# genomematt/xenomapper

Hardware: AMD Instinct MI355X
Metric: read-pairs/sec classified (higher is better)
Workload: dtype int32; 1 GPU; configs[1]: 50000000 PE 2x150 pairs/GPU, AS/XS, liberal, HBM-resident; pairs_per_gpu=50000000, step=xm_classify_compact_dev: classify+count, scan, scatter (3 launches)

## Files before the change

### xenomapper_amd/csrc/xm_kernels.hip

```cpp
#include <hip/hip_runtime.h>
#include <stdint.h>
#include <stdlib.h>

#include "xm_kernels.h"

namespace xm {

template <typename T>
__device__ __forceinline__ uint32_t mapping_state(T a1, T x1, T a2, T x2, T m)
{
    const bool low1 = a1 <= m;
    const bool low2 = a2 <= m;
    const bool prim = (a1 > m) && (low2 || a1 > a2);
    const bool sec  = (a2 > m) && (low1 || a2 > a1);
    const bool spec1 = (x1 == T(0)) || (a1 > x1);
    const bool spec2 = (x2 == T(0)) || (a2 > x2);
    uint32_t s = 6u;
    s = sec ? (spec2 ? 1u : 3u) : s;
    s = (a1 == a2) ? 4u : s;
    s = prim ? (spec1 ? 0u : 2u) : s;
    s = (low1 && low2) ? 5u : s;
    return s;
}

template <>
__device__ __forceinline__ uint32_t mapping_state<int32_t>(int32_t a1, int32_t x1, int32_t a2, int32_t x2, int32_t m)
{
    const bool low1 = a1 <= m, low2 = a2 <= m;
    const bool gt = a1 > a2, lt = a2 > a1;
    const bool spec1 = (x1 == 0) || (a1 > x1);
    const bool spec2 = (x2 == 0) || (a2 > x2);
    uint32_t s = spec2 ? 1u : 3u;
    s = (gt || lt) ? s : 4u;
    s = (!low1 && (low2 || gt)) ? (spec1 ? 0u : 2u) : s;
    s = (low1 && low2) ? 5u : s;
    return s;
}

__device__ __forceinline__ uint32_t bin_of_code(int mode, uint32_t c)
{
    const uint32_t f = (c >> 3) & 7u, r = c & 7u;
    const uint32_t lo = f < r ? f : r;
    const uint32_t hi = f < r ? r : f;
    uint32_t b;
    if (mode == XM_MODE_SE) {
        b = r > 6u ? 6u : r;
    } else if (mode == XM_MODE_PE_LIBERAL) {
        b = lo;
    } else {
        b = (hi == 5u) ? 5u
          : ((hi == 4u) || (((f ^ r) & 1u) != 0u)) ? 4u
          : lo;
    }
    if (mode != XM_MODE_SE) b = (hi > 5u) ? 6u : b;
    return (c == XM_NO_UNIT) ? 7u : b;
}

template <typename T> struct Vec4;
typedef int32_t v4i32 __attribute__((ext_vector_type(4)));
typedef int32_t v4i32_a4 __attribute__((ext_vector_type(4), aligned(4)));
typedef double  v4f64 __attribute__((ext_vector_type(4)));
template <> struct Vec4<int32_t> { typedef v4i32 type; };
template <> struct Vec4<double>  { typedef v4f64 type; };

template <typename T> __device__ __forceinline__ T absent_value();
template <> __device__ __forceinline__ int32_t absent_value<int32_t>() { return INT32_MIN; }
template <> __device__ __forceinline__ double  absent_value<double>()  { return -__builtin_huge_val(); }

template <typename T, bool NT, bool FULL = false>
__device__ __forceinline__ void load4(const T *__restrict__ col, uint64_t r0, uint64_t n, T out[4])
{
    typedef typename Vec4<T>::type V;
    if (FULL || r0 + 4 <= n) {
        const V *p = reinterpret_cast<const V *>(col + r0);
        const V v = NT ? __builtin_nontemporal_load(p) : *p;
        out[0] = v.x; out[1] = v.y; out[2] = v.z; out[3] = v.w;
    } else {
#pragma unroll
        for (int j = 0; j < 4; ++j) out[j] = (r0 + j < n) ? col[r0 + j] : absent_value<T>();
    }
}

template <typename T, bool NT>
__device__ __forceinline__ void load4_wg(const T *__restrict__ wg, uint32_t byte_off, T out[4])
{
    typedef typename Vec4<T>::type V;
    const V *p = reinterpret_cast<const V *>(reinterpret_cast<const char *>(wg) + byte_off);
    const V v = NT ? __builtin_nontemporal_load(p) : *p;
    out[0] = v.x; out[1] = v.y; out[2] = v.z; out[3] = v.w;
}

__device__ __forceinline__ uint32_t wave_scan_incl(uint32_t v)
{
    v += (uint32_t)__builtin_amdgcn_update_dpp(0, (int)v, 0x111, 0xf, 0xf, false);
    v += (uint32_t)__builtin_amdgcn_update_dpp(0, (int)v, 0x112, 0xf, 0xf, false);
    v += (uint32_t)__builtin_amdgcn_update_dpp(0, (int)v, 0x114, 0xf, 0xf, false);
    v += (uint32_t)__builtin_amdgcn_update_dpp(0, (int)v, 0x118, 0xf, 0xf, false);
    v += (uint32_t)__builtin_amdgcn_update_dpp(0, (int)v, 0x142, 0xa, 0xf, false);
    v += (uint32_t)__builtin_amdgcn_update_dpp(0, (int)v, 0x143, 0xc, 0xf, false);
    return v;
}

__device__ __forceinline__ uint32_t lane_value(uint32_t v, int lane)
{
    return (uint32_t)__builtin_amdgcn_readlane((int)v, lane);
}

__device__ __forceinline__ void lds_settle()
{
    asm volatile("s_waitcnt lgkmcnt(0)" ::: "memory");
}

#define XM_HREP 8
#define XM_COUNT_LDS_WORDS (64 * XM_HREP + 16)

struct CountSink {
    uint32_t *gran_counts;
    uint32_t *part_tot;
    unsigned long long *counts_rep;
    uint8_t *bins4;
    uint32_t gran_stride;
    int mode;
    uint32_t blk0;
};

__device__ __forceinline__ void count_flush(uint32_t *lds, uint32_t granule, const CountSink &sink)
{
    const uint32_t lane = threadIdx.x & 63u;
    uint32_t *misc = lds + 64 * XM_HREP;
    const uint4 h0 = *reinterpret_cast<const uint4 *>(lds + lane * XM_HREP);
    const uint4 h1 = *reinterpret_cast<const uint4 *>(lds + lane * XM_HREP + 4);
    const uint32_t s = h0.x + h0.y + h0.z + h0.w + h1.x + h1.y + h1.z + h1.w;
    if (s != 0u) {
        atomicAdd(&sink.counts_rep[(granule % XM_COUNT_REPLICAS) * 64u + lane], (unsigned long long)s);
        atomicAdd(&misc[8u + bin_of_code(sink.mode, lane)], s);
    }
    lds_settle();
    if (lane < 8u) {
        const uint32_t v = misc[8u + lane];
        sink.gran_counts[(uint64_t)lane * sink.gran_stride + granule] = v;
        if (v != 0u) atomicAdd(&sink.part_tot[((granule & (XM_PART_REPLICAS - 1u)) * 8u + lane) * XM_PART_STRIDE + granule / XM_PART_GRAN], v);
    }
}

template <int BLOCK>
__device__ __forceinline__ void count_units(const uint32_t c[4], uint32_t *lds, const CountSink &sink)
{
    const uint32_t lane = threadIdx.x & 63u;
    const uint32_t rep = lane & (XM_HREP - 1u);
#pragma unroll
    for (int j = 0; j < 4; ++j) {
        const bool unit = c[j] != XM_NO_UNIT;
        if (__ballot(unit) == 0ull) continue;
        if (unit) atomicAdd(&lds[(c[j] & 63u) * XM_HREP + rep], 1u);
    }
    lds_settle();
    uint32_t arrived = 0;
    if (lane == 0u) arrived = atomicAdd(&lds[64 * XM_HREP], 1u);
    arrived = (uint32_t)__builtin_amdgcn_readfirstlane((int)arrived);
    if (arrived != (uint32_t)(BLOCK / 64 - 1)) return;
    lds_settle();
    count_flush(lds, blockIdx.x + sink.blk0, sink);
}

template <int MODE, bool HAS6>
__device__ __forceinline__ uint32_t unit_bin(uint32_t c)
{
    if (MODE == XM_MODE_SE) return c == XM_NO_UNIT ? 7u : (c & 7u);
    const uint32_t f = (c >> 3) & 7u, r = c & 7u;
    const uint32_t lo = f < r ? f : r, hi = f < r ? r : f;
    uint32_t b = lo;
    if (MODE == XM_MODE_PE_CONSERVATIVE) {
        b = (((f ^ r) & 1u) != 0u || hi == 4u) ? 4u : b;
        b = (hi == 5u) ? 5u : b;
    }
    if (HAS6) b = (hi > 5u) ? 6u : b;
    return c == XM_NO_UNIT ? 7u : b;
}

template <int MODE, bool HAS6>
__device__ __forceinline__ uint32_t unit_bin_of(uint32_t f, uint32_t r, bool unit)
{
    uint32_t b;
    if (MODE == XM_MODE_SE) {
        b = r;
    } else {
        const uint32_t lo = f < r ? f : r, hi = f < r ? r : f;
        b = lo;
        if (MODE == XM_MODE_PE_CONSERVATIVE) {
            b = (((f ^ r) & 1u) != 0u || hi == 4u) ? 4u : b;
            b = (hi == 5u) ? 5u : b;
        }
        if (HAS6) b = (hi > 5u) ? 6u : b;
    }
    return unit ? b : 7u;
}

template <typename T, bool PAIRED, int BLOCK, bool FULL, bool COUNTS, int BINMODE>
__device__ __forceinline__ void classify_finish(const T a1[4], const T x1[4], const T a2[4], const T x2[4], T m,
                                                uint32_t mb, uint32_t halo, uint32_t *last_state,
                                                uint8_t *__restrict__ code, uint64_t r0, uint64_t n,
                                                uint32_t *count_lds, const CountSink &sink)
{
    const uint32_t lane = threadIdx.x & 63u;
    const uint32_t wave = threadIdx.x >> 6;
    uint32_t s[4];
#pragma unroll
    for (int j = 0; j < 4; ++j) s[j] = mapping_state<T>(a1[j], x1[j], a2[j], x2[j], m);

    uint32_t c[4], fwd[4] = {0, 0, 0, 0};
    if (PAIRED) {
        uint32_t prev = (uint32_t)__builtin_amdgcn_update_dpp(0, (int)s[3], 0x138, 0xf, 0xf, false);
        if (lane == 63) last_state[wave] = s[3];
        __syncthreads();
        if (lane == 0) prev = (wave == 0) ? halo : last_state[wave - 1];
        c[0] = (mb & 1u) ? ((prev << 3) | s[0]) : XM_NO_UNIT;
        c[1] = (mb & 2u) ? ((s[0] << 3) | s[1]) : XM_NO_UNIT;
        c[2] = (mb & 4u) ? ((s[1] << 3) | s[2]) : XM_NO_UNIT;
        c[3] = (mb & 8u) ? ((s[2] << 3) | s[3]) : XM_NO_UNIT;
        fwd[0] = prev; fwd[1] = s[0]; fwd[2] = s[1]; fwd[3] = s[2];
    } else {
        if (COUNTS) __syncthreads();
#pragma unroll
        for (int j = 0; j < 4; ++j) c[j] = ((mb >> j) & 1u) ? s[j] : XM_NO_UNIT;
    }

    if (FULL || r0 + 4 <= n) {
        if (code != nullptr) *reinterpret_cast<uint32_t *>(code + r0) = c[0] | (c[1] << 8) | (c[2] << 16) | (c[3] << 24);
    } else {
#pragma unroll
        for (int j = 0; j < 4; ++j)
            if (code != nullptr && r0 + j < n) code[r0 + j] = (uint8_t)c[j];
    }
    if (BINMODE >= 0) {
        uint32_t nib = 0;
#pragma unroll
        for (int j = 0; j < 4; ++j) nib |= unit_bin_of<BINMODE, sizeof(T) == 8>(fwd[j], s[j], ((mb >> j) & 1u) != 0u) << (4 * j);
        reinterpret_cast<uint16_t *>(sink.bins4)[r0 >> 2] = (uint16_t)nib;
    }
    if (COUNTS) count_units<BLOCK>(c, count_lds, sink);
}

template <typename T, bool PAIRED, bool NT, int BLOCK, bool FULL, bool COUNTS, int BINMODE>
__device__ __forceinline__ void classify_body(const T *__restrict__ as1, const T *__restrict__ xs1,
                                              const T *__restrict__ as2, const T *__restrict__ xs2,
                                              const uint8_t *__restrict__ unit_bits8, T m,
                                              uint8_t *__restrict__ code, uint64_t n, uint32_t *last_state,
                                              uint32_t *count_lds, const CountSink &sink)
{
    const uint64_t g = (uint64_t)(blockIdx.x + sink.blk0) * BLOCK + threadIdx.x;
    const uint64_t r0 = g * 4;

    T a1[4], x1[4], a2[4], x2[4];
    load4<T, NT, FULL>(as1, r0, n, a1);
    load4<T, NT, FULL>(xs1, r0, n, x1);
    load4<T, NT, FULL>(as2, r0, n, a2);
    load4<T, NT, FULL>(xs2, r0, n, x2);
    uint32_t mb = 0;
    if (FULL || r0 < n) mb = (uint32_t)(unit_bits8[g >> 1] >> ((g & 1u) * 4u)) & 0xFu;
    if (!FULL && r0 + 4 > n) mb &= (r0 < n) ? ((1u << (uint32_t)(n - r0)) - 1u) : 0u;

    uint32_t halo = 0;
    if (PAIRED && threadIdx.x == 0) {
        if (r0 > 0) {
            const uint64_t h = r0 - 1;
            halo = mapping_state<T>(as1[h], xs1[h], as2[h], xs2[h], m);
        } else {
            mb &= ~1u;
        }
    }
    classify_finish<T, PAIRED, BLOCK, FULL, COUNTS, BINMODE>(a1, x1, a2, x2, m, mb, halo, last_state, code, r0, n, count_lds, sink);
}

template <int BLOCK>
__device__ __forceinline__ void count_lds_clear(uint32_t *count_lds)
{
    for (uint32_t k = threadIdx.x; k < (uint32_t)XM_COUNT_LDS_WORDS; k += BLOCK) count_lds[k] = 0;
}

template <typename T, bool PAIRED, bool NT, int BLOCK, bool COUNTS, int BINMODE>
__global__ void __launch_bounds__(BLOCK)
classify_kernel(const T *__restrict__ as1, const T *__restrict__ xs1,
                const T *__restrict__ as2, const T *__restrict__ xs2,
                const uint8_t *__restrict__ unit_bits8, T m,
                uint8_t *__restrict__ code, uint64_t n, CountSink sink)
{
    __shared__ uint32_t last_state[BLOCK / 64];
    __shared__ __attribute__((aligned(16))) uint32_t count_lds[COUNTS ? XM_COUNT_LDS_WORDS : 4];
    if (COUNTS) count_lds_clear<BLOCK>(count_lds);
    if (((uint64_t)blockIdx.x + sink.blk0 + 1) * (BLOCK * 4) <= n)
        classify_body<T, PAIRED, NT, BLOCK, true, COUNTS, BINMODE>(as1, xs1, as2, xs2, unit_bits8, m, code, n, last_state, count_lds, sink);
    else
        classify_body<T, PAIRED, NT, BLOCK, false, COUNTS, BINMODE>(as1, xs1, as2, xs2, unit_bits8, m, code, n, last_state, count_lds, sink);
}


__device__ __attribute__((noinline)) uint4 load_codes16_tail(const uint8_t *__restrict__ code, uint64_t base, uint64_t n)
{
    uint32_t w[4];
    for (int k = 0; k < 4; ++k) {
        uint32_t acc = 0;
        for (int j = 0; j < 4; ++j) {
            const uint64_t i = base + 4 * k + j;
            const uint32_t c = (i < n) ? (uint32_t)code[i] : XM_NO_UNIT;
            acc |= c << (8 * j);
        }
        w[k] = acc;
    }
    return make_uint4(w[0], w[1], w[2], w[3]);
}

__device__ __forceinline__ void load_codes16(const uint8_t *__restrict__ code, uint64_t base, uint64_t n,
                                             uint32_t w[4])
{
    uint4 v;
    if (base + 16 <= n) v = *reinterpret_cast<const uint4 *>(code + base);
    else v = load_codes16_tail(code, base, n);
    w[0] = v.x; w[1] = v.y; w[2] = v.z; w[3] = v.w;
}

__device__ __attribute__((noinline)) uint32_t load_codes4_tail(const uint8_t *__restrict__ code, uint64_t base, uint64_t n)
{
    uint32_t acc = 0;
    for (int j = 0; j < 4; ++j) {
        const uint64_t i = base + j;
        const uint32_t c = (i < n) ? (uint32_t)code[i] : XM_NO_UNIT;
        acc |= c << (8 * j);
    }
    return acc;
}

__global__ void __launch_bounds__(XM_BLOCK)
hist_kernel(const uint8_t *__restrict__ code, uint64_t n, uint32_t n_gran, CountSink sink)
{
    __shared__ __attribute__((aligned(16))) uint32_t lds_all[XM_BLOCK / 64][XM_COUNT_LDS_WORDS];
    const uint32_t lane = threadIdx.x & 63u, wave = threadIdx.x >> 6;
    uint32_t *lds = lds_all[wave];
    const uint32_t g = blockIdx.x * (XM_BLOCK / 64) + wave;
    if (g >= n_gran) return;
    for (uint32_t k = lane; k < (uint32_t)XM_COUNT_LDS_WORDS; k += 64u) lds[k] = 0;

    constexpr int TILES = XM_GRAN / 1024;
    const uint64_t rec0 = (uint64_t)g * XM_GRAN;
    uint32_t w[TILES][4];
#pragma unroll
    for (int k = 0; k < TILES; ++k) load_codes16(code, rec0 + (uint64_t)k * 1024u + lane * 16u, n, w[k]);
    lds_settle();

    const uint32_t rep = lane & (XM_HREP - 1u);
    uint32_t common = w[0][0] & 0xFFu;
    if (common == XM_NO_UNIT) common = (w[0][0] >> 8) & 0xFFu;
    common = (uint32_t)__builtin_amdgcn_readfirstlane((int)common);
    uint32_t n_common = 0;
#pragma unroll
    for (int k = 0; k < TILES; ++k) {
#pragma unroll
        for (int j = 0; j < 16; ++j) {
            const uint32_t c = (w[k][j >> 2] >> (8 * (j & 3))) & 0xFFu;
            const bool unit = c != XM_NO_UNIT;
            if (__ballot(unit) == 0ull) continue;
            const bool same = unit && c == common;
            n_common += same ? 1u : 0u;
            if (unit && !same) atomicAdd(&lds[(c & 63u) * XM_HREP + rep], 1u);
        }
    }
    if (n_common) atomicAdd(&lds[(common & 63u) * XM_HREP + rep], n_common);
    lds_settle();
    count_flush(lds, g, sink);
}

#define XM_SCAN_THREADS 1024
__device__ __forceinline__ unsigned long long block_sum_1024(unsigned long long v, unsigned long long *wsum)
{
    v += __shfl_xor(v, 1, 64);  v += __shfl_xor(v, 2, 64);  v += __shfl_xor(v, 4, 64);
    v += __shfl_xor(v, 8, 64);  v += __shfl_xor(v, 16, 64); v += __shfl_xor(v, 32, 64);
    if ((threadIdx.x & 63u) == 0u) wsum[threadIdx.x >> 6] = v;
    __syncthreads();
    unsigned long long total = 0;
#pragma unroll
    for (int w = 0; w < XM_SCAN_THREADS / 64; ++w) total += wsum[w];
    return total;
}

__global__ void __launch_bounds__(XM_SCAN_THREADS)
scan_kernel(const uint32_t *__restrict__ gran_counts, uint32_t n_gran, uint32_t gran_stride,
            const uint32_t *__restrict__ part_tot, uint32_t *__restrict__ gran_off,
            unsigned long long *__restrict__ bin_totals,
            unsigned long long *__restrict__ counts_rep, unsigned long long *__restrict__ counts, uint32_t part0, uint32_t n_parts)
{
    __shared__ unsigned long long wsum[XM_SCAN_THREADS / 64];
    __shared__ uint32_t wtot[XM_SCAN_THREADS / 64];
    const uint32_t p = blockIdx.x + part0, b = blockIdx.y;
    const uint32_t t = threadIdx.x, lane = t & 63u, wave = t >> 6;
    if (p + 1u == n_parts && t < 64u) {
        const uint32_t slot = b * 8u + (t >> 3), part = t & 7u;
        unsigned long long acc = 0;
        for (uint32_t r = part; r < XM_COUNT_REPLICAS; r += 8u) {
            acc += counts_rep[r * 64u + slot];
            counts_rep[r * 64u + slot] = 0;
        }
        acc += __shfl_xor(acc, 1, 64);
        acc += __shfl_xor(acc, 2, 64);
        acc += __shfl_xor(acc, 4, 64);
        if (part == 0) counts[slot] = acc;
    }
    const uint32_t g = p * XM_PART_GRAN + t;
    const uint32_t x = (g < n_gran) ? gran_counts[(uint64_t)b * gran_stride + g] : 0u;
    unsigned long long part_sum = 0;
    for (uint32_t e = t; e < p * XM_PART_REPLICAS; e += XM_SCAN_THREADS) {
        const uint32_t r = e / p, q = e - r * p;
        part_sum += part_tot[(r * 8u + b) * XM_PART_STRIDE + q];
    }
    const unsigned long long carry = block_sum_1024(part_sum, wsum);

    const uint32_t incl = wave_scan_incl(x);
    if (lane == 63u) wtot[wave] = incl;
    __syncthreads();
    uint32_t before_wave = 0, part_total = 0;
    for (uint32_t w = 0; w < XM_SCAN_THREADS / 64; ++w) {
        const uint32_t v = wtot[w];
        before_wave += (w < wave) ? v : 0u;
        part_total += v;
    }
    if (g < n_gran) gran_off[(uint64_t)b * gran_stride + g] = (uint32_t)carry + before_wave + incl - x;
    if (p + 1u == n_parts && t == 0u) bin_totals[b] = carry + part_total;
}

#ifndef XM_SCATTER_GUARD
#define XM_SCATTER_GUARD 1
#endif
__device__ __forceinline__ uint32_t mbcnt64(uint64_t mask, uint32_t add)
{
    return __builtin_amdgcn_mbcnt_hi((uint32_t)(mask >> 32), __builtin_amdgcn_mbcnt_lo((uint32_t)mask, add));
}

template <bool WIDE>
__device__ __forceinline__ void store_index(uint32_t *__restrict__ idx_out, uint32_t pos, uint32_t rec)
{
    if (WIDE) idx_out[pos] = rec;
    else *reinterpret_cast<uint32_t *>(reinterpret_cast<char *>(idx_out) + (pos << 2)) = rec;
}

template <int SLOTS, bool WIDE, bool STAGED, bool LISTS = false>
__device__ __forceinline__ void scatter_256(const uint32_t bin[4], const uint32_t rec[4], uint32_t base[7],
                                            uint32_t *__restrict__ idx_out, uint32_t n_units, uint16_t *slab,
                                            const uint64_t *lptr = nullptr)
{
    uint32_t pos[4] = {0, 0, 0, 0};
#pragma unroll
    for (int b = 0; b < 7; ++b) {
        uint64_t m[4], any = 0;
#pragma unroll
        for (int j = 0; j < 4; ++j) {
            m[j] = ((SLOTS >> j) & 1) ? __ballot(bin[j] == (uint32_t)b) : 0ull;
            any |= m[j];
        }
        if (any == 0ull) continue;
        uint32_t t = base[b];
#pragma unroll
        for (int j = 0; j < 4; ++j)
            if ((SLOTS >> j) & 1) t = mbcnt64(m[j], t);
#pragma unroll
        for (int j = 0; j < 4; ++j)
            if ((SLOTS >> j) & 1) pos[j] = (bin[j] == (uint32_t)b) ? t : pos[j];
        uint32_t total = 0;
#pragma unroll
        for (int j = 0; j < 4; ++j)
            if ((SLOTS >> j) & 1) total += (uint32_t)__builtin_popcountll(m[j]);
        base[b] += total;
    }
#pragma unroll
    for (int j = 1; j < 4; ++j)
#pragma unroll
        for (int i = 0; i < j; ++i)
            if (((SLOTS >> j) & 1) && ((SLOTS >> i) & 1)) pos[j] += (bin[i] == bin[j]) ? 1u : 0u;
#pragma unroll
    for (int j = 0; j < 4; ++j)
        if (((SLOTS >> j) & 1) && bin[j] < 7u && (!XM_SCATTER_GUARD || pos[j] < n_units)) {
            if (STAGED) slab[pos[j]] = (uint16_t)rec[j];
            else if (LISTS) {
                uint32_t *list = reinterpret_cast<uint32_t *>(lptr[bin[j]]);
                if (list != nullptr) list[pos[j]] = rec[j];
            }
            else store_index<WIDE>(idx_out, pos[j], rec[j]);
        }
}

#ifndef XM_SCATTER_STAGED
#define XM_SCATTER_STAGED 1
#endif
#define XM_SLAB_U16 (XM_GRAN + 64)
#ifndef XM_STAGE_MIN_UNITS
#define XM_STAGE_MIN_UNITS 1536
#endif

template <bool WIDE>
__device__ __forceinline__ void store_index4(uint32_t *__restrict__ idx_out, uint32_t pos, uint32_t r0, uint32_t r1, uint32_t r2, uint32_t r3)
{
    typedef uint32_t v4u32_a4 __attribute__((ext_vector_type(4), aligned(4)));
    v4u32_a4 v; v.x = r0; v.y = r1; v.z = r2; v.w = r3;
    if (WIDE) *reinterpret_cast<v4u32_a4 *>(idx_out + pos) = v;
    else *reinterpret_cast<v4u32_a4 *>(reinterpret_cast<char *>(idx_out) + (pos << 2)) = v;
}

template <bool WIDE>
__device__ __forceinline__ void scatter_copy_out(const uint16_t *slab, uint32_t L, uint32_t G, uint32_t N, uint32_t rec_g,
                                                 uint32_t *__restrict__ idx_out)
{
    const uint32_t lane = threadIdx.x & 63u;
    if (N < 64u) {
        if (lane < N) store_index<WIDE>(idx_out, G + lane, rec_g + slab[L + lane]);
        return;
    }
    const uint32_t h = (0u - G) & 3u;
    const uint32_t body = (N - h) >> 2;
    const uint32_t t = (N - h) & 3u;
    {
        const bool head = lane < h, tail = lane >= 4u && lane - 4u < t;
        const uint32_t e = head ? lane : h + 4u * body + (lane - 4u);
        if (head || tail) store_index<WIDE>(idx_out, G + e, rec_g + slab[L + e]);
    }
    for (uint32_t c = lane; c < body; c += 64u) {
        const uint32_t e = h + 4u * c;
        const uint2 w = *reinterpret_cast<const uint2 *>(slab + L + e);
        store_index4<WIDE>(idx_out, G + e, rec_g + (w.x & 0xFFFFu), rec_g + (w.x >> 16), rec_g + (w.y & 0xFFFFu), rec_g + (w.y >> 16));
    }
}

template <int NSUB, bool WIDE, bool NIB, bool STAGED, bool LISTS>
__device__ __forceinline__ void scatter_granule(const uint32_t w[NSUB], const uint8_t *lut, uint32_t rec_g, uint32_t base[7],
                                                uint32_t *__restrict__ idx_out, uint32_t n_units, uint16_t *slab, const uint64_t *lptr)
{
    const uint32_t lane = threadIdx.x & 63u;
#pragma unroll
    for (int s = 0; s < NSUB; ++s) {
        const uint32_t rec0 = (STAGED ? 0u : rec_g) + (uint32_t)s * 256u + lane * 4u;
        const uint32_t limit = STAGED ? (uint32_t)XM_SLAB_U16 : n_units;
        uint32_t bin[4];
        bool even_free;
        if (NIB) {
#pragma unroll
            for (int j = 0; j < 4; ++j) bin[j] = (w[s] >> (4 * j)) & 7u;
            even_free = (w[s] & 0x0707u) == 0x0707u;
        } else {
            even_free = (w[s] & 0x00FF00FFu) == 0x00FF00FFu;
        }
        const uint32_t rec[4] = {rec0, rec0 + 1u, rec0 + 2u, rec0 + 3u};
        if (__ballot(!even_free) == 0ull) {
            if (!NIB) { bin[0] = bin[2] = 7u; bin[1] = lut[(w[s] >> 8) & 63u]; bin[3] = lut[(w[s] >> 24) & 63u]; }
            scatter_256<0xA, WIDE, STAGED, LISTS && !STAGED>(bin, rec, base, idx_out, limit, slab, lptr);
            continue;
        }
        if (!NIB) {
#pragma unroll
            for (int j = 0; j < 4; ++j) bin[j] = lut[(w[s] >> (8 * j)) & 63u];
        }
        uint32_t y;
        if (NIB) {
            const uint32_t x = w[s] ^ 0x7777u;
            y = (x | (x >> 1) | (x >> 2)) & 0x1111u;
        } else {
            y = (bin[0] < 7u ? 1u : 0u) | (bin[1] < 7u ? 0x10u : 0u) | (bin[2] < 7u ? 0x100u : 0u) | (bin[3] < 7u ? 0x1000u : 0u);
        }
        if (!STAGED && __ballot(__builtin_popcount(y) > 2) == 0ull) {
            const uint32_t rest = y & (y - 1u);
            const uint32_t c0 = y ? (uint32_t)__builtin_ctz(y) : 0u, c1 = rest ? (uint32_t)__builtin_ctz(rest) : 0u;
            const uint32_t j0 = c0 >> 2, j1 = c1 >> 2;
            uint32_t vb[4] = {7u, 7u, 7u, 7u};
            if (NIB) {
                vb[0] = y ? (w[s] >> c0) & 7u : 7u;
                vb[1] = rest ? (w[s] >> c1) & 7u : 7u;
            } else {
#pragma unroll
                for (int j = 0; j < 4; ++j) {
                    vb[0] = (y && j0 == (uint32_t)j) ? bin[j] : vb[0];
                    vb[1] = (rest && j1 == (uint32_t)j) ? bin[j] : vb[1];
                }
            }
            const uint32_t vrec[4] = {rec0 + j0, rec0 + j1, 0u, 0u};
            scatter_256<0x3, WIDE, STAGED, LISTS>(vb, vrec, base, idx_out, limit, slab, lptr);
        } else {
            scatter_256<0xF, WIDE, STAGED, LISTS && !STAGED>(bin, rec, base, idx_out, limit, slab, lptr);
        }
    }
}

template <int NSUB, bool WIDE, bool NIB, bool STAGE, bool LISTS, bool MULTI>
__global__ void __launch_bounds__(XM_BLOCK)
scatter_kernel(const uint8_t *__restrict__ code, uint64_t n, int mode, uint32_t n_gran, uint32_t gran_stride,
               const uint32_t *__restrict__ gran_counts, const uint32_t *__restrict__ gran_off,
               const unsigned long long *__restrict__ bin_totals,
               unsigned long long *__restrict__ bin_offsets, uint32_t *__restrict__ idx_out, uint32_t *__restrict__ part_tot,
               const ListOut lo, uint32_t gran_per_wave, uint32_t g_first, uint32_t last)
{
    constexpr bool CAN_STAGE = STAGE && XM_SCATTER_STAGED != 0 && NSUB * 256 == XM_GRAN;
    __shared__ uint8_t lut_all[NIB ? 1 : XM_BLOCK / 64][64];
    __shared__ uint64_t lptr_all[LISTS ? XM_BLOCK / 64 : 1][8];
    __shared__ __attribute__((aligned(16))) uint16_t slab_all[CAN_STAGE ? XM_BLOCK / 64 : 1][CAN_STAGE ? XM_SLAB_U16 : 4];
    const uint32_t lane = threadIdx.x & 63u;
    if (last) {
        const uint32_t n_parts = (n_gran + XM_PART_GRAN - 1u) / XM_PART_GRAN, cells = 8u * XM_PART_REPLICAS * n_parts;
        for (uint32_t i = blockIdx.x * XM_BLOCK + threadIdx.x; i < cells; i += gridDim.x * XM_BLOCK)
            part_tot[(i / n_parts) * XM_PART_STRIDE + i % n_parts] = 0u;
    }
    const uint32_t wave = (uint32_t)__builtin_amdgcn_readfirstlane((int)(threadIdx.x >> 6));
    const uint32_t g0 = g_first + (blockIdx.x * (XM_BLOCK / 64) + wave) * (MULTI ? gran_per_wave : 1u);
    if (g0 >= n_gran) return;
    uint8_t *lut = lut_all[NIB ? 0 : wave];
    if (!NIB) lut[lane] = (uint8_t)bin_of_code(mode, lane == 63u ? XM_NO_UNIT : lane);
    uint64_t *lptr = lptr_all[LISTS ? wave : 0];
    if (LISTS && lane < 8u) lptr[lane] = lane < 7u ? (uint64_t)(uintptr_t)lo.p[lane] : 0ull;

    uint32_t lane_base, n_units;
    {
        const uint32_t tot = (lane < 8u) ? (uint32_t)bin_totals[lane] : 0u;
        const uint32_t off = (lane < 7u) ? gran_off[(uint64_t)lane * gran_stride + g0] : 0u;
        const uint32_t bin_start = wave_scan_incl(tot) - tot;
        lane_base = LISTS ? off : bin_start + off;
        n_units = LISTS ? lo.cap : lane_value(bin_start, 7);
        if (g0 == g_first && last && lane < 8u) bin_offsets[lane] = (LISTS && lane < 7u) ? tot : bin_start;
    }
    uint16_t *slab = slab_all[CAN_STAGE ? wave : 0];

    auto load_granule = [&](uint32_t g, uint32_t w[NSUB]) {
        const uint64_t rec_g = (uint64_t)g * (NSUB * 256u);
        if (NIB) {
            const uint16_t *nib = reinterpret_cast<const uint16_t *>(code) + (rec_g >> 2) + lane;
#pragma unroll
            for (int s = 0; s < NSUB; ++s) w[s] = nib[s * 64];
        } else if (rec_g + NSUB * 256u <= n) {
#pragma unroll
            for (int s = 0; s < NSUB; ++s) w[s] = *reinterpret_cast<const uint32_t *>(code + rec_g + s * 256u + lane * 4u);
        } else {
#pragma unroll
            for (int s = 0; s < NSUB; ++s) w[s] = load_codes4_tail(code, rec_g + s * 256u + lane * 4u, n);
        }
    };
    auto slab_layout = [&](uint32_t cnt_g, uint32_t &run_start, uint32_t &run_len) -> bool {
        const uint32_t room = (lane < 7u) ? ((cnt_g + 3u) & ~3u) + 4u : 0u;
        const uint32_t incl_room = wave_scan_incl(room), incl_cnt = wave_scan_incl(cnt_g);
        run_start = incl_room - room + (lane_base & 3u);
        const uint32_t cnt = lane_base < n_units ? (cnt_g < n_units - lane_base ? cnt_g : n_units - lane_base) : 0u;
        run_len = run_start < (uint32_t)XM_SLAB_U16 ? (cnt < XM_SLAB_U16 - run_start ? cnt : XM_SLAB_U16 - run_start) : 0u;
        return lane_value(incl_cnt, 6) >= (uint32_t)XM_STAGE_MIN_UNITS;
    };
    auto copy_runs_out = [&](uint32_t run_start, uint32_t run_len, uint32_t rec_g) {
#pragma unroll
        for (int b = 0; b < 7; ++b) {
            const uint32_t N = lane_value(run_len, b);
            uint32_t *__restrict__ dst = LISTS ? lo.p[b] : idx_out;
            if (N == 0u || dst == nullptr) continue;
            scatter_copy_out<WIDE>(slab, lane_value(run_start, b), lane_value(lane_base, b), N, rec_g, dst);
        }
    };

    if (!MULTI) {
        const uint32_t g = g0;
        uint32_t run_start = 0, run_len = 0;
        bool staged = false;
        if (CAN_STAGE) {
            const uint32_t cnt_g = (lane < 7u) ? gran_counts[(uint64_t)lane * gran_stride + g] : 0u;
            staged = slab_layout(cnt_g, run_start, run_len);
        }
        uint32_t base[7];
#pragma unroll
        for (int b = 0; b < 7; ++b) base[b] = lane_value(staged ? run_start : lane_base, b);
        const uint32_t rec_g = (uint32_t)((uint64_t)g * (NSUB * 256u));
        uint32_t w[NSUB];
        load_granule(g, w);
        if (!NIB || LISTS) lds_settle();
        if (CAN_STAGE && staged) {
            scatter_granule<NSUB, WIDE, NIB, true, LISTS>(w, lut, rec_g, base, idx_out, n_units, slab, lptr);
            lds_settle();
            copy_runs_out(run_start, run_len, rec_g);
        } else {
            scatter_granule<NSUB, WIDE, NIB, false, LISTS>(w, lut, rec_g, base, idx_out, n_units, slab, lptr);
        }
        return;
    }

    const uint32_t g1 = g0 + gran_per_wave < n_gran ? g0 + gran_per_wave : n_gran;
    uint32_t base[7];
#pragma unroll
    for (int b = 0; b < 7; ++b) base[b] = lane_value(lane_base, b);
    uint32_t w[NSUB], wn[NSUB];
    load_granule(g0, w);
    if (!NIB || LISTS) lds_settle();
    for (uint32_t g = g0; g < g1; ++g) {
        if (g + 1u < g1) load_granule(g + 1u, wn);
        const uint32_t rec_g = (uint32_t)((uint64_t)g * (NSUB * 256u));
        bool staged = false;
        uint32_t cnt_g = 0;
        if (CAN_STAGE) {
            cnt_g = (lane < 7u) ? gran_counts[(uint64_t)lane * gran_stride + g] : 0u;
            uint32_t run_start, run_len;
            staged = slab_layout(cnt_g, run_start, run_len);
            if (staged) {
                uint32_t sbase[7];
#pragma unroll
                for (int b = 0; b < 7; ++b) sbase[b] = lane_value(run_start, b);
                scatter_granule<NSUB, WIDE, NIB, true, LISTS>(w, lut, rec_g, sbase, idx_out, n_units, slab, lptr);
                lds_settle();
                copy_runs_out(run_start, run_len, rec_g);
                lds_settle();
            }
        }
        if (!staged) {
            if (CAN_STAGE) {
#pragma unroll
                for (int b = 0; b < 7; ++b) base[b] = lane_value(lane_base, b);
            }
            scatter_granule<NSUB, WIDE, NIB, false, LISTS>(w, lut, rec_g, base, idx_out, n_units, slab, lptr);
        }
        if (CAN_STAGE) lane_base += cnt_g;
#pragma unroll
        for (int s = 0; s < NSUB; ++s) w[s] = wn[s];
    }
}

#define XM_RUNS_WCNT_AT (64 * XM_HREP)
#define XM_RUNS_SLAB_AT (XM_RUNS_WCNT_AT + 64)
#define XM_RUNS_LDS_WORDS (XM_RUNS_SLAB_AT + XM_GRAN / 2)

struct RunsSink {
    uint16_t *runs16;
    uint16_t *gran_counts16;
    unsigned long long *counts_rep;
};

template <int SLOTS, int NB>
__device__ __forceinline__ uint32_t runs_ranks(const uint32_t bin[4], uint32_t pos[4])
{
    const uint32_t lane = threadIdx.x & 63u;
    uint32_t wc = 0;
#pragma unroll
    for (int b = 0; b < NB; ++b) {
        uint64_t m[4], any = 0;
#pragma unroll
        for (int j = 0; j < 4; ++j) {
            m[j] = ((SLOTS >> j) & 1) ? __ballot(bin[j] == (uint32_t)b) : 0ull;
            any |= m[j];
        }
        if (any == 0ull) continue;
        uint32_t t = 0, total = 0;
#pragma unroll
        for (int j = 0; j < 4; ++j)
            if ((SLOTS >> j) & 1) { t = mbcnt64(m[j], t); total += (uint32_t)__builtin_popcountll(m[j]); }
#pragma unroll
        for (int j = 0; j < 4; ++j)
            if ((SLOTS >> j) & 1) pos[j] = (bin[j] == (uint32_t)b) ? t : pos[j];
        wc = (lane == (uint32_t)b) ? total : wc;
    }
#pragma unroll
    for (int j = 1; j < 4; ++j)
#pragma unroll
        for (int i = 0; i < j; ++i)
            if (((SLOTS >> j) & 1) && ((SLOTS >> i) & 1)) pos[j] += (bin[i] == bin[j]) ? 1u : 0u;
    return wc;
}

template <typename T, bool PAIRED, bool NT, int BLOCK, bool FULL, int BINMODE>
__device__ __forceinline__ void classify_runs_body(const T *__restrict__ as1, const T *__restrict__ xs1,
                                                   const T *__restrict__ as2, const T *__restrict__ xs2,
                                                   const uint8_t *__restrict__ unit_bits8, T m, uint64_t n,
                                                   uint32_t *last_state, uint32_t *lds, const RunsSink &rs)
{
    static_assert(BLOCK == 512 && BLOCK * 4 == XM_GRAN, "eight waves, one granule");
    constexpr bool HAS6 = sizeof(T) == 8;
    constexpr int NB = HAS6 ? 7 : 6;
    const uint32_t lane = threadIdx.x & 63u;
    const uint32_t wave = (uint32_t)__builtin_amdgcn_readfirstlane((int)(threadIdx.x >> 6));
    const uint32_t g = blockIdx.x;
    const uint64_t g4 = (uint64_t)blockIdx.x * BLOCK + threadIdx.x;
    const uint64_t r0 = g4 * 4;
    T a1[4], x1[4], a2[4], x2[4];
    load4<T, NT, FULL>(as1, r0, n, a1);
    load4<T, NT, FULL>(xs1, r0, n, x1);
    load4<T, NT, FULL>(as2, r0, n, a2);
    load4<T, NT, FULL>(xs2, r0, n, x2);
    uint32_t mb = 0;
    if (FULL || r0 < n) mb = (uint32_t)(unit_bits8[g4 >> 1] >> ((g4 & 1u) * 4u)) & 0xFu;
    if (!FULL && r0 + 4 > n) mb &= (r0 < n) ? ((1u << (uint32_t)(n - r0)) - 1u) : 0u;
    uint32_t halo = 0;
    if (PAIRED && threadIdx.x == 0) {
        if (r0 > 0) {
            const uint64_t h = r0 - 1;
            halo = mapping_state<T>(as1[h], xs1[h], as2[h], xs2[h], m);
        } else {
            mb &= ~1u;
        }
    }
    uint32_t s[4];
#pragma unroll
    for (int j = 0; j < 4; ++j) s[j] = mapping_state<T>(a1[j], x1[j], a2[j], x2[j], m);
    uint32_t c[4], fwd[4] = {0, 0, 0, 0};
    if (PAIRED) {
        uint32_t prev = (uint32_t)__builtin_amdgcn_update_dpp(0, (int)s[3], 0x138, 0xf, 0xf, false);
        if (lane == 63) last_state[wave] = s[3];
        __syncthreads();
        if (lane == 0) prev = (wave == 0) ? halo : last_state[wave - 1];
        c[0] = (mb & 1u) ? ((prev << 3) | s[0]) : XM_NO_UNIT;
        c[1] = (mb & 2u) ? ((s[0] << 3) | s[1]) : XM_NO_UNIT;
        c[2] = (mb & 4u) ? ((s[1] << 3) | s[2]) : XM_NO_UNIT;
        c[3] = (mb & 8u) ? ((s[2] << 3) | s[3]) : XM_NO_UNIT;
        fwd[0] = prev; fwd[1] = s[0]; fwd[2] = s[1]; fwd[3] = s[2];
    } else {
        __syncthreads();
#pragma unroll
        for (int j = 0; j < 4; ++j) c[j] = ((mb >> j) & 1u) ? s[j] : XM_NO_UNIT;
    }
    uint32_t bin[4];
#pragma unroll
    for (int j = 0; j < 4; ++j) bin[j] = unit_bin_of<BINMODE, HAS6>(fwd[j], s[j], ((mb >> j) & 1u) != 0u);
    {
        const uint32_t rep = lane & (XM_HREP - 1u);
#pragma unroll
        for (int j = 0; j < 4; ++j) {
            const bool unit = c[j] != XM_NO_UNIT;
            if (__ballot(unit) == 0ull) continue;
            if (unit) atomicAdd(&lds[(c[j] & 63u) * XM_HREP + rep], 1u);
        }
    }
    uint32_t pos[4] = {0, 0, 0, 0};
    const bool inter = PAIRED && __ballot((mb & 5u) != 0u) == 0ull;
    const uint32_t wc = inter ? runs_ranks<0xA, NB>(bin, pos) : runs_ranks<0xF, NB>(bin, pos);
    uint32_t *wave_cnt = lds + XM_RUNS_WCNT_AT;
    uint16_t *slab = reinterpret_cast<uint16_t *>(lds + XM_RUNS_SLAB_AT);
    if (lane < 8u) wave_cnt[wave * 8u + lane] = wc;
    __syncthreads();
    uint32_t off, tot;
    {
        const uint32_t v = wave_cnt[lane];
        off = (lane >> 3) < wave ? v : 0u;
        tot = v;
        off += (uint32_t)__shfl_xor((int)off, 8, 64);  tot += (uint32_t)__shfl_xor((int)tot, 8, 64);
        off += (uint32_t)__shfl_xor((int)off, 16, 64); tot += (uint32_t)__shfl_xor((int)tot, 16, 64);
        off += (uint32_t)__shfl_xor((int)off, 32, 64); tot += (uint32_t)__shfl_xor((int)tot, 32, 64);
    }
    const uint32_t t8 = lane < 8u ? tot : 0u;
    const uint32_t incl8 = wave_scan_incl(t8);
    const uint32_t where = incl8 - t8 + off;
    const uint32_t units = lane_value(incl8, 7);
#pragma unroll
    for (int j = 0; j < 4; ++j) {
        uint32_t at = 0;
#pragma unroll
        for (int b = 0; b < NB; ++b) at = (bin[j] == (uint32_t)b) ? lane_value(where, b) : at;
        if (bin[j] < 7u) slab[at + pos[j]] = (uint16_t)(threadIdx.x * 4u + (uint32_t)j);
    }
    __syncthreads();
    if (threadIdx.x < (uint32_t)(XM_GRAN / 8) && threadIdx.x * 8u < units)
        reinterpret_cast<uint4 *>(rs.runs16 + (uint64_t)g * XM_GRAN)[threadIdx.x] = reinterpret_cast<const uint4 *>(slab)[threadIdx.x];
    if (wave == 0u) {
        if (lane < 8u) rs.gran_counts16[(uint64_t)g * 8u + lane] = (uint16_t)tot;
        const uint4 h0 = *reinterpret_cast<const uint4 *>(lds + lane * XM_HREP);
        const uint4 h1 = *reinterpret_cast<const uint4 *>(lds + lane * XM_HREP + 4);
        const uint32_t sum = h0.x + h0.y + h0.z + h0.w + h1.x + h1.y + h1.z + h1.w;
        if (sum != 0u) atomicAdd(&rs.counts_rep[(g % XM_COUNT_REPLICAS) * 64u + lane], (unsigned long long)sum);
    }
}

template <typename T, bool PAIRED, bool NT, int BLOCK, int BINMODE>
__global__ void __launch_bounds__(BLOCK)
classify_runs_kernel(const T *__restrict__ as1, const T *__restrict__ xs1, const T *__restrict__ as2, const T *__restrict__ xs2,
                     const uint8_t *__restrict__ unit_bits8, T m, uint64_t n, RunsSink rs)
{
    __shared__ uint32_t last_state[BLOCK / 64];
    __shared__ __attribute__((aligned(16))) uint32_t lds[XM_RUNS_LDS_WORDS];
    for (uint32_t q = threadIdx.x; q < 64u * XM_HREP; q += BLOCK) lds[q] = 0;
    if (((uint64_t)blockIdx.x + 1) * (BLOCK * 4) <= n)
        classify_runs_body<T, PAIRED, NT, BLOCK, true, BINMODE>(as1, xs1, as2, xs2, unit_bits8, m, n, last_state, lds, rs);
    else
        classify_runs_body<T, PAIRED, NT, BLOCK, false, BINMODE>(as1, xs1, as2, xs2, unit_bits8, m, n, last_state, lds, rs);
}

__global__ void __launch_bounds__(256)
runs_finish_kernel(unsigned long long *__restrict__ counts_rep, unsigned long long *__restrict__ counts,
                   unsigned long long *__restrict__ n_out, int mode)
{
    __shared__ unsigned long long part[4][64];
    __shared__ unsigned long long bins[8];
    const uint32_t slot = threadIdx.x & 63u, q = threadIdx.x >> 6;
    unsigned long long acc = 0;
#pragma unroll
    for (uint32_t r = 0; r < XM_COUNT_REPLICAS / 4u; ++r) {
        acc += counts_rep[(q * (XM_COUNT_REPLICAS / 4u) + r) * 64u + slot];
        counts_rep[(q * (XM_COUNT_REPLICAS / 4u) + r) * 64u + slot] = 0;
    }
    part[q][slot] = acc;
    if (threadIdx.x < 8u) bins[threadIdx.x] = 0;
    __syncthreads();
    if (q == 0u) {
        const unsigned long long v = part[0][slot] + part[1][slot] + part[2][slot] + part[3][slot];
        counts[slot] = v;
        if (v != 0ull) {
            atomicAdd(&bins[bin_of_code(mode, slot)], v);
            atomicAdd(&bins[7], v);
        }
    }
    __syncthreads();
    if (threadIdx.x < 8u) n_out[threadIdx.x] = bins[threadIdx.x];
}

__global__ void __launch_bounds__(XM_BLOCK)
cigar_kernel(uint64_t n, const int32_t *__restrict__ nm, const uint32_t *__restrict__ cig_off,
             const uint32_t *__restrict__ cig_oplen, int32_t *__restrict__ as_out,
             uint32_t *__restrict__ range_flag)
{
    const uint64_t stride = (uint64_t)gridDim.x * XM_BLOCK;
    for (uint64_t i = (uint64_t)blockIdx.x * XM_BLOCK + threadIdx.x; i < n; i += stride) {
        const int32_t nmv = nm[i];
        int32_t out = INT32_MIN;
        if (nmv != INT32_MIN) {
            long long s = -6ll * (long long)nmv;
            const uint32_t k1 = cig_off[i + 1];
            for (uint32_t k = cig_off[i]; k < k1; ++k) {
                const uint32_t v = cig_oplen[k];
                const uint32_t op = v & 15u;
                const long long len = (long long)(v >> 4);
                s -= (op == 1u || op == 2u) ? (5ll + 3ll * len) : 0ll;
                s -= (op == 4u) ? 2ll * len : 0ll;
            }
            if (s <= (long long)INT32_MIN || s > (long long)INT32_MAX) {
                if (range_flag) atomicOr(range_flag, 1u);
                s = s < 0 ? (long long)INT32_MIN + 1 : (long long)INT32_MAX;
            }
            out = (int32_t)s;
        }
        as_out[i] = out;
    }
}

#define XM_CIG_SPEC 3

__device__ __forceinline__ long long cigar_term(uint32_t v)
{
    const uint32_t op = v & 15u;
    const long long len = (long long)(v >> 4);
    long long t = (op == 1u || op == 2u) ? (5ll + 3ll * len) : 0ll;
    t += (op == 4u) ? 2ll * len : 0ll;
    return t;
}

__device__ __forceinline__ uint32_t cigar_term32(uint32_t v)
{
    const uint32_t op = v & 15u, len = v >> 4;
    uint32_t t = (op == 1u || op == 2u) ? (5u + 3u * len) : 0u;
    t += (op == 4u) ? 2u * len : 0u;
    return t;
}

__device__ __forceinline__ uint32_t cigar_term24(uint32_t v)
{
    uint32_t op = v & 15u;
    op = op < 8u ? op : 8u;
    const uint32_t a = __builtin_amdgcn_ubfe(0x00000550u, op * 4u, 4u);
    const uint32_t b = __builtin_amdgcn_ubfe(0x00020330u, op * 4u, 4u);
    return __umul24(b, v >> 4) + a;
}

__device__ __forceinline__ int32_t cigar_clamp(long long s, uint32_t *range_flag)
{
    if (s <= (long long)INT32_MIN || s > (long long)INT32_MAX) {
        if (range_flag) atomicOr(range_flag, 1u);
        s = s < 0 ? (long long)INT32_MIN + 1 : (long long)INT32_MAX;
    }
    return (int32_t)s;
}

__device__ __forceinline__ int32_t cigar_score_one(const int32_t *__restrict__ nm, const uint32_t *__restrict__ off,
                                                   const uint32_t *__restrict__ ops, uint64_t i, uint32_t *range_flag)
{
    const int32_t nmv = nm[i];
    if (nmv == INT32_MIN) return INT32_MIN;
    long long s = -6ll * (long long)nmv;
    const uint32_t k1 = off[i + 1];
    for (uint32_t k = off[i]; k < k1; ++k) s -= cigar_term(ops[k]);
    return cigar_clamp(s, range_flag);
}

struct __attribute__((packed, aligned(4))) Ops3 {
    uint32_t v[XM_CIG_SPEC];
};

template <bool FULL>
__device__ __forceinline__ void cigar_fetch_offsets(const int32_t *__restrict__ nm, const uint32_t *__restrict__ off,
                                                    uint64_t r0, uint64_t n, int32_t nmv[4], uint32_t o[5])
{
    load4<int32_t, true, FULL>(nm, r0, n, nmv);
    if (FULL || r0 + 4 <= n) {
        const v4i32 q = __builtin_nontemporal_load(reinterpret_cast<const v4i32 *>(off + r0));
        o[0] = (uint32_t)q.x; o[1] = (uint32_t)q.y; o[2] = (uint32_t)q.z; o[3] = (uint32_t)q.w;
        o[4] = off[r0 + 4];
    } else {
        uint32_t prev = 0u;
#pragma unroll
        for (int j = 0; j < 5; ++j) {
            const uint32_t v = (r0 + j <= n) ? off[r0 + j] : prev;
            o[j] = v;
            prev = v;
        }
    }
}

__device__ __forceinline__ void cigar_fetch_ops(const uint32_t *__restrict__ ops, uint32_t n_ops, const uint32_t o[5],
                                                uint32_t v[4][XM_CIG_SPEC])
{
    if (__ballot(o[3] + XM_CIG_SPEC > n_ops) == 0ull) {
#pragma unroll
        for (int j = 0; j < 4; ++j) {
            const Ops3 t = *reinterpret_cast<const Ops3 *>(ops + o[j]);
#pragma unroll
            for (int q = 0; q < XM_CIG_SPEC; ++q) v[j][q] = t.v[q];
        }
    } else {
#pragma unroll
        for (int j = 0; j < 4; ++j)
#pragma unroll
            for (int q = 0; q < XM_CIG_SPEC; ++q) v[j][q] = (o[j] + (uint32_t)q < o[j + 1]) ? ops[o[j] + q] : 0u;
    }
}

__device__ __forceinline__ bool cigar_finish_scores(const uint32_t *__restrict__ ops, const int32_t nmv[4], const uint32_t o[5],
                                                    const uint32_t v[4][XM_CIG_SPEC], int32_t as_out[4])
{
    long long s[4];
    bool longer = false;
#pragma unroll
    for (int j = 0; j < 4; ++j) {
        const uint32_t k = o[j + 1] - o[j];
        uint32_t acc = 0;
#pragma unroll
        for (int q = 0; q < XM_CIG_SPEC; ++q) acc += ((uint32_t)q < k) ? cigar_term32(v[j][q]) : 0u;
        s[j] = -6ll * (long long)nmv[j] - (long long)acc;
        longer |= k > (uint32_t)XM_CIG_SPEC;
    }
    if (__ballot(longer) != 0ull) {
#pragma unroll
        for (int j = 0; j < 4; ++j)
            for (uint32_t k = o[j] + XM_CIG_SPEC; k < o[j + 1]; ++k) s[j] -= cigar_term(ops[k]);
    }
    bool bad = false;
#pragma unroll
    for (int j = 0; j < 4; ++j) {
        const bool present = nmv[j] != INT32_MIN;
        const bool out = present && (s[j] <= (long long)INT32_MIN || s[j] > (long long)INT32_MAX);
        bad |= out;
        const long long c = out ? (s[j] < 0 ? (long long)INT32_MIN + 1 : (long long)INT32_MAX) : s[j];
        as_out[j] = present ? (int32_t)c : INT32_MIN;
    }
    return bad;
}

#define XM_CIG_WAVE_OPS 1024
__device__ __forceinline__ bool cigar_scores_by_prefix(const uint32_t *__restrict__ ops, uint32_t n_ops, const int32_t nmv[4],
                                                       const uint32_t o[5], uint32_t *T, int32_t as_out[4], bool &bad)
{
    const uint32_t lane = threadIdx.x & 63u;
    const uint32_t base = __builtin_amdgcn_readfirstlane(o[0]);
    const uint32_t W = lane_value(o[4], 63) - base;
    bool odd = false;
#pragma unroll
    for (int j = 0; j < 4; ++j) odd |= (o[j + 1] - o[j]) > 512u;
    if (W >= (uint32_t)XM_CIG_WAVE_OPS || __ballot(odd) != 0ull) return false;
    uint32_t carry = 0;
    const uint32_t chunks = W / 256u + 1u;
    for (uint32_t c = 0; c < chunks; ++c) {
        const uint32_t s0 = c * 256u + 4u * lane;
        uint32_t v[4];
        if (base + (c + 1u) * 256u <= n_ops) {
            v[0] = v[1] = v[2] = v[3] = 0u;
            if (s0 < W) {
                const v4i32 q = *reinterpret_cast<const v4i32_a4 *>(ops + base + s0);
                v[0] = (uint32_t)q.x; v[1] = (uint32_t)q.y; v[2] = (uint32_t)q.z; v[3] = (uint32_t)q.w;
            }
        } else {
#pragma unroll
            for (int q = 0; q < 4; ++q) v[q] = (base + s0 + (uint32_t)q < n_ops) ? ops[base + s0 + (uint32_t)q] : 0u;
        }
        uint32_t t[4];
#pragma unroll
        for (int q = 0; q < 4; ++q) {
            const bool in = s0 + (uint32_t)q < W;
            odd |= in && (v[q] >> 4) >= (1u << 20);
            t[q] = in ? cigar_term32(v[q]) : 0u;
        }
        const uint32_t p1 = t[0], p2 = p1 + t[1], p3 = p2 + t[2], tot = p3 + t[3];
        const uint32_t incl = wave_scan_incl(tot);
        const uint32_t ex = incl - tot + carry;
        *reinterpret_cast<uint4 *>(T + s0) = make_uint4(ex, ex + p1, ex + p2, ex + p3);
        carry += lane_value(incl, 63);
    }
    if (__ballot(odd) != 0ull) return false;
#pragma unroll
// ... 618 lines not shown
```

Measured before the change: 142.5 billion read-pairs/s.

## Hoist and batch global loads across classify, scan and scatter kernels

The classify kernels now issue the halo element loads for the preceding row up front, uniformly per workgroup, so they overlap the main vector loads instead of running as a serialized thread-0 branch afterwards. The scan kernel loads the replica counts and the first few partial-total cells into registers before reducing them, and moves the replica-count close to the end. The scatter kernel prefetches the granule codes, totals, offsets, counts and list pointers together before one explicit vmem waitcnt, and prefetches the next granule's count in the loop. Together these increase memory-level parallelism at the cost of more registers, redundant halo loads in every lane, and explicit full vmem waits.

```diff
diff --git a/xenomapper_amd/csrc/xm_kernels.hip b/xenomapper_amd/csrc/xm_kernels.hip
--- a/xenomapper_amd/csrc/xm_kernels.hip
+++ b/xenomapper_amd/csrc/xm_kernels.hip
@@ -109,6 +109,11 @@
 __device__ __forceinline__ void lds_settle()
 {
     asm volatile("s_waitcnt lgkmcnt(0)" ::: "memory");
+}
+
+__device__ __forceinline__ void vmem_settle()
+{
+    __builtin_amdgcn_s_waitcnt(0x0F70);
 }
 
 #define XM_HREP 8
@@ -251,6 +256,11 @@
     const uint64_t g = (uint64_t)(blockIdx.x + sink.blk0) * BLOCK + threadIdx.x;
     const uint64_t r0 = g * 4;
 
+    const uint64_t wg_r0 = (uint64_t)(blockIdx.x + sink.blk0) * (BLOCK * 4);
+    const bool has_halo = PAIRED && wg_r0 > 0;
+    T ha1 = T(0), hx1 = T(0), ha2 = T(0), hx2 = T(0);
+    if (has_halo) { ha1 = as1[wg_r0 - 1]; hx1 = xs1[wg_r0 - 1]; ha2 = as2[wg_r0 - 1]; hx2 = xs2[wg_r0 - 1]; }
+
     T a1[4], x1[4], a2[4], x2[4];
     load4<T, NT, FULL>(as1, r0, n, a1);
     load4<T, NT, FULL>(xs1, r0, n, x1);
@@ -261,14 +271,8 @@
     if (!FULL && r0 + 4 > n) mb &= (r0 < n) ? ((1u << (uint32_t)(n - r0)) - 1u) : 0u;
 
     uint32_t halo = 0;
-    if (PAIRED && threadIdx.x == 0) {
-        if (r0 > 0) {
-            const uint64_t h = r0 - 1;
-            halo = mapping_state<T>(as1[h], xs1[h], as2[h], xs2[h], m);
-        } else {
-            mb &= ~1u;
-        }
-    }
+    if (has_halo) halo = mapping_state<T>(ha1, hx1, ha2, hx2, m);
+    else if (PAIRED && threadIdx.x == 0) mb &= ~1u;
     classify_finish<T, PAIRED, BLOCK, FULL, COUNTS, BINMODE>(a1, x1, a2, x2, m, mb, halo, last_state, code, r0, n, count_lds, sink);
 }
 
@@ -370,6 +374,7 @@
 }
 
 #define XM_SCAN_THREADS 1024
+#define XM_SCAN_CARRY_AHEAD 4u
 __device__ __forceinline__ unsigned long long block_sum_1024(unsigned long long v, unsigned long long *wsum)
 {
     v += __shfl_xor(v, 1, 64);  v += __shfl_xor(v, 2, 64);  v += __shfl_xor(v, 4, 64);
@@ -392,25 +397,35 @@
     __shared__ uint32_t wtot[XM_SCAN_THREADS / 64];
     const uint32_t p = blockIdx.x + part0, b = blockIdx.y;
     const uint32_t t = threadIdx.x, lane = t & 63u, wave = t >> 6;
-    if (p + 1u == n_parts && t < 64u) {
-        const uint32_t slot = b * 8u + (t >> 3), part = t & 7u;
-        unsigned long long acc = 0;
-        for (uint32_t r = part; r < XM_COUNT_REPLICAS; r += 8u) {
-            acc += counts_rep[r * 64u + slot];
-            counts_rep[r * 64u + slot] = 0;
-        }
-        acc += __shfl_xor(acc, 1, 64);
-        acc += __shfl_xor(acc, 2, 64);
-        acc += __shfl_xor(acc, 4, 64);
-        if (part == 0) counts[slot] = acc;
+    constexpr uint32_t REP_PER_LANE = XM_COUNT_REPLICAS / 8u;
+    const bool closes = p + 1u == n_parts && t < 64u;
+    const uint32_t slot = b * 8u + ((t >> 3) & 7u), piece = t & 7u;
+    unsigned long long rep[REP_PER_LANE];
+#pragma unroll
+    for (uint32_t k = 0; k < REP_PER_LANE; ++k) rep[k] = 0;
+    if (closes) {
+#pragma unroll
+        for (uint32_t k = 0; k < REP_PER_LANE; ++k) rep[k] = counts_rep[(piece + 8u * k) * 64u + slot];
+    }
+    const uint32_t cells = p * XM_PART_REPLICAS, pdiv = p ? p : 1u;
+    auto part_cell = [&](uint32_t e) -> const uint32_t * {
+        const uint32_t r = e / pdiv, q = e - r * pdiv;
+        return part_tot + (r * 8u + b) * XM_PART_STRIDE + q;
+    };
+    uint32_t ahead[XM_SCAN_CARRY_AHEAD];
+#pragma unroll
+    for (uint32_t k = 0; k < XM_SCAN_CARRY_AHEAD; ++k) {
+        const uint32_t e = t + k * XM_SCAN_THREADS;
+        ahead[k] = *part_cell(e < cells ? e : 0u);
     }
     const uint32_t g = p * XM_PART_GRAN + t;
-    const uint32_t x = (g < n_gran) ? gran_counts[(uint64_t)b * gran_stride + g] : 0u;
+    const uint32_t x_any = gran_counts[(uint64_t)b * gran_stride + (g < n_gran ? g : 0u)];
+    const uint32_t x = (g < n_gran) ? x_any : 0u;
     unsigned long long part_sum = 0;
-    for (uint32_t e = t; e < p * XM_PART_REPLICAS; e += XM_SCAN_THREADS) {
-        const uint32_t r = e / p, q = e - r * p;
-        part_sum += part_tot[(r * 8u + b) * XM_PART_STRIDE + q];
-    }
+#pragma unroll
+    for (uint32_t k = 0; k < XM_SCAN_CARRY_AHEAD; ++k) part_sum += (t + k * XM_SCAN_THREADS < cells) ? ahead[k] : 0u;
+    for (uint32_t e = t + XM_SCAN_CARRY_AHEAD * XM_SCAN_THREADS; e < cells; e += XM_SCAN_THREADS)
+        part_sum += *part_cell(e);
     const unsigned long long carry = block_sum_1024(part_sum, wsum);
 
     const uint32_t incl = wave_scan_incl(x);
@@ -424,6 +439,18 @@
     }
     if (g < n_gran) gran_off[(uint64_t)b * gran_stride + g] = (uint32_t)carry + before_wave + incl - x;
     if (p + 1u == n_parts && t == 0u) bin_totals[b] = carry + part_total;
+    if (closes) {
+        unsigned long long acc = 0;
+#pragma unroll
+        for (uint32_t k = 0; k < REP_PER_LANE; ++k) {
+            acc += rep[k];
+            counts_rep[(piece + 8u * k) * 64u + slot] = 0;
+        }
+        acc += __shfl_xor(acc, 1, 64);
+        acc += __shfl_xor(acc, 2, 64);
+        acc += __shfl_xor(acc, 4, 64);
+        if (piece == 0) counts[slot] = acc;
+    }
 }
 
 #ifndef XM_SCATTER_GUARD
@@ -598,44 +625,55 @@
     __shared__ uint64_t lptr_all[LISTS ? XM_BLOCK / 64 : 1][8];
     __shared__ __attribute__((aligned(16))) uint16_t slab_all[CAN_STAGE ? XM_BLOCK / 64 : 1][CAN_STAGE ? XM_SLAB_U16 : 4];
     const uint32_t lane = threadIdx.x & 63u;
-    if (last) {
+    auto zero_part_totals = [&]() {
+        if (!last) return;
         const uint32_t n_parts = (n_gran + XM_PART_GRAN - 1u) / XM_PART_GRAN, cells = 8u * XM_PART_REPLICAS * n_parts;
         for (uint32_t i = blockIdx.x * XM_BLOCK + threadIdx.x; i < cells; i += gridDim.x * XM_BLOCK)
             part_tot[(i / n_parts) * XM_PART_STRIDE + i % n_parts] = 0u;
-    }
+    };
     const uint32_t wave = (uint32_t)__builtin_amdgcn_readfirstlane((int)(threadIdx.x >> 6));
     const uint32_t g0 = g_first + (blockIdx.x * (XM_BLOCK / 64) + wave) * (MULTI ? gran_per_wave : 1u);
-    if (g0 >= n_gran) return;
+    if (g0 >= n_gran) { zero_part_totals(); return; }
     uint8_t *lut = lut_all[NIB ? 0 : wave];
     if (!NIB) lut[lane] = (uint8_t)bin_of_code(mode, lane == 63u ? XM_NO_UNIT : lane);
     uint64_t *lptr = lptr_all[LISTS ? wave : 0];
-    if (LISTS && lane < 8u) lptr[lane] = lane < 7u ? (uint64_t)(uintptr_t)lo.p[lane] : 0ull;
-
+    uint16_t *slab = slab_all[CAN_STAGE ? wave : 0];
+
+    auto load_granule = [&](uint32_t g, uint32_t w[NSUB]) {
+        const uint64_t rec_g = (uint64_t)g * (NSUB * 256u);
+        if (NIB) {
+            const uint16_t *nib = reinterpret_cast<const uint16_t *>(code) + (rec_g >> 2) + lane;
+#pragma unroll
+            for (int s = 0; s < NSUB; ++s) w[s] = nib[s * 64];
+        } else if (rec_g + NSUB * 256u <= n) {
+#pragma unroll
+            for (int s = 0; s < NSUB; ++s) w[s] = *reinterpret_cast<const uint32_t *>(code + rec_g + s * 256u + lane * 4u);
+        } else {
+#pragma unroll
+            for (int s = 0; s < NSUB; ++s) w[s] = load_codes4_tail(code, rec_g + s * 256u + lane * 4u, n);
+        }
+    };
+    auto load_count = [&](uint32_t g) -> uint32_t {
+        return (CAN_STAGE && lane < 7u) ? gran_counts[(uint64_t)lane * gran_stride + g] : 0u;
+    };
+
+    uint32_t w[NSUB];
+    load_granule(g0, w);
+    const uint32_t tot = (lane < 8u) ? (uint32_t)bin_totals[lane] : 0u;
+    const uint32_t off = (lane < 7u) ? gran_off[(uint64_t)lane * gran_stride + g0] : 0u;
+    const uint32_t cnt0 = load_count(g0);
+    const uint64_t my_list = (LISTS && lane < 7u) ? (uint64_t)(uintptr_t)lo.p[lane] : 0ull;
+    vmem_settle();
+    if (LISTS && lane < 8u) lptr[lane] = my_list;
+    zero_part_totals();
     uint32_t lane_base, n_units;
     {
-        const uint32_t tot = (lane < 8u) ? (uint32_t)bin_totals[lane] : 0u;
-        const uint32_t off = (lane < 7u) ? gran_off[(uint64_t)lane * gran_stride + g0] : 0u;
         const uint32_t bin_start = wave_scan_incl(tot) - tot;
         lane_base = LISTS ? off : bin_start + off;
         n_units = LISTS ? lo.cap : lane_value(bin_start, 7);
         if (g0 == g_first && last && lane < 8u) bin_offsets[lane] = (LISTS && lane < 7u) ? tot : bin_start;
     }
-    uint16_t *slab = slab_all[CAN_STAGE ? wave : 0];
-
-    auto load_granule = [&](uint32_t g, uint32_t w[NSUB]) {
-        const uint64_t rec_g = (uint64_t)g * (NSUB * 256u);
-        if (NIB) {
-            const uint16_t *nib = reinterpret_cast<const uint16_t *>(code) + (rec_g >> 2) + lane;
-#pragma unroll
-            for (int s = 0; s < NSUB; ++s) w[s] = nib[s * 64];
-        } else if (rec_g + NSUB * 256u <= n) {
-#pragma unroll
-            for (int s = 0; s < NSUB; ++s) w[s] = *reinterpret_cast<const uint32_t *>(code + rec_g + s * 256u + lane * 4u);
-        } else {
-#pragma unroll
-            for (int s = 0; s < NSUB; ++s) w[s] = load_codes4_tail(code, rec_g + s * 256u + lane * 4u, n);
-        }
-    };
+
     auto slab_layout = [&](uint32_t cnt_g, uint32_t &run_start, uint32_t &run_len) -> bool {
         const uint32_t room = (lane < 7u) ? ((cnt_g + 3u) & ~3u) + 4u : 0u;
         const uint32_t incl_room = wave_scan_incl(room), incl_cnt = wave_scan_incl(cnt_g);
@@ -658,16 +696,11 @@
         const uint32_t g = g0;
         uint32_t run_start = 0, run_len = 0;
         bool staged = false;
-        if (CAN_STAGE) {
-            const uint32_t cnt_g = (lane < 7u) ? gran_counts[(uint64_t)lane * gran_stride + g] : 0u;
-            staged = slab_layout(cnt_g, run_start, run_len);
-        }
+        if (CAN_STAGE) staged = slab_layout(cnt0, run_start, run_len);
         uint32_t base[7];
 #pragma unroll
         for (int b = 0; b < 7; ++b) base[b] = lane_value(staged ? run_start : lane_base, b);
         const uint32_t rec_g = (uint32_t)((uint64_t)g * (NSUB * 256u));
-        uint32_t w[NSUB];
-        load_granule(g, w);
         if (!NIB || LISTS) lds_settle();
         if (CAN_STAGE && staged) {
             scatter_granule<NSUB, WIDE, NIB, true, LISTS>(w, lut, rec_g, base, idx_out, n_units, slab, lptr);
@@ -683,16 +716,18 @@
     uint32_t base[7];
 #pragma unroll
     for (int b = 0; b < 7; ++b) base[b] = lane_value(lane_base, b);
-    uint32_t w[NSUB], wn[NSUB];
-    load_granule(g0, w);
+    uint32_t wn[NSUB], cnt_g = cnt0;
     if (!NIB || LISTS) lds_settle();
     for (uint32_t g = g0; g < g1; ++g) {
-        if (g + 1u < g1) load_granule(g + 1u, wn);
+        uint32_t cnt_n = 0;
+        if (g + 1u < g1) {
+            load_granule(g + 1u, wn);
+            cnt_n = load_count(g + 1u);
+            vmem_settle();
+        }
         const uint32_t rec_g = (uint32_t)((uint64_t)g * (NSUB * 256u));
         bool staged = false;
-        uint32_t cnt_g = 0;
         if (CAN_STAGE) {
-            cnt_g = (lane < 7u) ? gran_counts[(uint64_t)lane * gran_stride + g] : 0u;
             uint32_t run_start, run_len;
             staged = slab_layout(cnt_g, run_start, run_len);
             if (staged) {
@@ -713,6 +748,7 @@
             scatter_granule<NSUB, WIDE, NIB, false, LISTS>(w, lut, rec_g, base, idx_out, n_units, slab, lptr);
         }
         if (CAN_STAGE) lane_base += cnt_g;
+        cnt_g = cnt_n;
 #pragma unroll
         for (int s = 0; s < NSUB; ++s) w[s] = wn[s];
     }
@@ -773,6 +809,10 @@
     const uint32_t g = blockIdx.x;
     const uint64_t g4 = (uint64_t)blockIdx.x * BLOCK + threadIdx.x;
     const uint64_t r0 = g4 * 4;
+    const uint64_t wg_r0 = (uint64_t)blockIdx.x * (BLOCK * 4);
+    const bool has_halo = PAIRED && wg_r0 > 0;
+    T ha1 = T(0), hx1 = T(0), ha2 = T(0), hx2 = T(0);
+    if (has_halo) { ha1 = as1[wg_r0 - 1]; hx1 = xs1[wg_r0 - 1]; ha2 = as2[wg_r0 - 1]; hx2 = xs2[wg_r0 - 1]; }
     T a1[4], x1[4], a2[4], x2[4];
     load4<T, NT, FULL>(as1, r0, n, a1);
     load4<T, NT, FULL>(xs1, r0, n, x1);
@@ -782,14 +822,8 @@
     if (FULL || r0 < n) mb = (uint32_t)(unit_bits8[g4 >> 1] >> ((g4 & 1u) * 4u)) & 0xFu;
     if (!FULL && r0 + 4 > n) mb &= (r0 < n) ? ((1u << (uint32_t)(n - r0)) - 1u) : 0u;
     uint32_t halo = 0;
-    if (PAIRED && threadIdx.x == 0) {
-        if (r0 > 0) {
-            const uint64_t h = r0 - 1;
-            halo = mapping_state<T>(as1[h], xs1[h], as2[h], xs2[h], m);
-        } else {
-            mb &= ~1u;
-        }
-    }
+    if (has_halo) halo = mapping_state<T>(ha1, hx1, ha2, hx2, m);
+    else if (PAIRED && threadIdx.x == 0) mb &= ~1u;
     uint32_t s[4];
 #pragma unroll
     for (int j = 0; j < 4; ++j) s[j] = mapping_state<T>(a1[j], x1[j], a2[j], x2[j], m);
```

After: 124.1 billion read-pairs/s. -12.9%, worse.
